# ucla-brain/image-preprocessing-pipeline

Hardware: AMD Instinct MI355X
Metric: RL-deconv Gvoxels/sec (higher is better)
Workload: dtype f32; 1 GPU; c3: 2048x2048x512 fp32 volume, 31x31x61 PSF, deconFFT semantics, lambda=0, reg_interval=0; engine=fft, parallelism=single

## Files before the change

image-preprocessing-pipeline_amd/csrc/fft_native_dev.h:

```cpp
#pragma once
#include <cmath>
#include <cstdlib>
#include <type_traits>
#include <vector>

#include "fft_native.h"

namespace mi {
namespace {

#ifndef MI_FFT_UNROLL
#define MI_FFT_UNROLL 4
#endif
#ifndef MI_YCUT
#define MI_YCUT 1
#endif
constexpr int kYCut = MI_YCUT;

__host__ __device__ constexpr int swz_g(int t) { return ((t & 1) ? 15 : 0) ^ ((t & 2) ? 13 : 0) ^ ((t & 4) ? 25 : 0) ^ ((t & 8) ? 16 : 0); }
__host__ __device__ constexpr int swz_c(int i) { return i ^ swz_g((i >> 4) & 15); }
__host__ __device__ constexpr unsigned long long swz_table_hi() {
    unsigned long long v = 0;
    for (int t = 0; t < 8; ++t) v |= (unsigned long long)swz_g(2 * t) << (5 * t);
    return v;
}
__device__ __forceinline__ int phys(int i) {
    constexpr unsigned long long T = swz_table_hi();
    const int hi = (int)((T >> (5 * ((i >> 5) & 7))) & 31ull);
    return i ^ hi ^ (__builtin_amdgcn_sbfe(i, 4, 1) & 15);
}
constexpr int kRowsRot = 256;
__device__ __forceinline__ int rmask(int row, int hp) {
    if (hp & kRowsRot) return (row >> 1) & ((hp & (kRowsRot - 1)) - 1);
    const int rp = (row >> 1) & (hp - 1);
    const int s = hp == 8 ? 1 : hp == 4 ? 2 : hp == 2 ? 3 : 0;
    return (rp << s) ^ ((rp & 1) << 4);
}

__device__ __forceinline__ int launder(int x) {
    asm volatile("" : "+v"(x));
    return x;
}
__device__ __forceinline__ void lds_barrier() {
    __builtin_amdgcn_fence(__ATOMIC_RELEASE, "workgroup", "local");
    __builtin_amdgcn_s_barrier();
    __builtin_amdgcn_fence(__ATOMIC_ACQUIRE, "workgroup", "local");
}
__device__ __forceinline__ void wave_lds_fence() {
    __builtin_amdgcn_fence(__ATOMIC_RELEASE, "wavefront", "local");
    __builtin_amdgcn_fence(__ATOMIC_ACQUIRE, "wavefront", "local");
}

__device__ __forceinline__ void stage_sync(bool priv) {
    if (priv) wave_lds_fence();
    else lds_barrier();
}

__device__ __forceinline__ float rcp_eps(float c) { return __builtin_amdgcn_rcpf(fmaxf(c, kEpsSingle)); }

typedef float v2f __attribute__((ext_vector_type(2)));
__device__ __forceinline__ v2f V2(float2 a) { return v2f{a.x, a.y}; }
__device__ __forceinline__ float2 F2(v2f a) { return make_float2(a.x, a.y); }
__device__ __forceinline__ float2 cmul(float2 a, float2 b) {
    const v2f A = V2(a), B = V2(b);
    const v2f axx = __builtin_shufflevector(A, A, 0, 0), ayy = __builtin_shufflevector(A, A, 1, 1);
    const v2f bs = {-B.y, B.x};
    return F2(__builtin_elementwise_fma(ayy, bs, axx * B));
}
__device__ __forceinline__ float2 cmulc(float2 a, float2 b) {
    const v2f A = V2(a), B = V2(b);
    const v2f axx = __builtin_shufflevector(A, A, 0, 0), ayy = __builtin_shufflevector(A, A, 1, 1);
    const v2f bc = {B.x, -B.y}, bsw = {B.y, B.x};
    return F2(__builtin_elementwise_fma(ayy, bsw, axx * bc));
}
__device__ __forceinline__ float2 cadd(float2 a, float2 b) { return F2(V2(a) + V2(b)); }
__device__ __forceinline__ float2 csub(float2 a, float2 b) { return F2(V2(a) - V2(b)); }
__device__ __forceinline__ float2 cconj(float2 a) { return make_float2(a.x, -a.y); }
__device__ __forceinline__ unsigned brev_n(unsigned v, int bits) { return bits == 0 ? 0u : (__brev(v) >> (32 - bits)); }

__device__ __forceinline__ int pos2freq(int p, int l2, int r3) {
    const int k1 = p >> l2, pp = p & ((1 << l2) - 1);
    return k1 + r3 * (int)brev_n((unsigned)pp, l2);
}
__device__ __forceinline__ int freq2pos(int k, int l2, int r3) {
    const int k2 = k / r3, k1 = k - k2 * r3;
    return (k1 << l2) + (int)brev_n((unsigned)k2, l2);
// ... 280 lines not shown
            dft3<INVERSE>(v[0], v[1], v[2]);
        } else if constexpr (R3 == 5) {
            dft5<INVERSE>(v);
        } else {
            if constexpr (!INVERSE) {
#pragma unroll
                for (int r = 0; r < 3; ++r) dft3<false>(v[r], v[r + 3], v[r + 6]);
                const float c9[3] = {1.0f, 0.76604444311897801f, 0.17364817766693033f};
                const float s9[3] = {0.0f, 0.64278760968653933f, 0.98480775301220802f};
                const float c94 = -0.93969262078590843f, s94 = 0.34202014332566871f;
                v[4] = cmul(v[4], make_float2(c9[1], -s9[1]));
                v[7] = cmul(v[7], make_float2(c9[2], -s9[2]));
                v[5] = cmul(v[5], make_float2(c9[2], -s9[2]));
                v[8] = cmul(v[8], make_float2(c94, -s94));
#pragma unroll
                for (int k1 = 0; k1 < 3; ++k1) dft3<false>(v[3 * k1], v[3 * k1 + 1], v[3 * k1 + 2]);
                float2 t[9];
#pragma unroll
                for (int k1 = 0; k1 < 3; ++k1)
#pragma unroll
                    for (int k2 = 0; k2 < 3; ++k2) t[k1 + 3 * k2] = v[3 * k1 + k2];
#pragma unroll
                for (int q = 0; q < 9; ++q) v[q] = t[q];
            } else {
                float2 t[9];
#pragma unroll
                for (int k1 = 0; k1 < 3; ++k1)
#pragma unroll
                    for (int k2 = 0; k2 < 3; ++k2) t[3 * k1 + k2] = v[k1 + 3 * k2];
#pragma unroll
                for (int q = 0; q < 9; ++q) v[q] = t[q];
#pragma unroll
                for (int k1 = 0; k1 < 3; ++k1) dft3<true>(v[3 * k1], v[3 * k1 + 1], v[3 * k1 + 2]);
                const float c9[3] = {1.0f, 0.76604444311897801f, 0.17364817766693033f};
                const float s9[3] = {0.0f, 0.64278760968653933f, 0.98480775301220802f};
                const float c94 = -0.93969262078590843f, s94 = 0.34202014332566871f;
                v[4] = cmul(v[4], make_float2(c9[1], s9[1]));
                v[7] = cmul(v[7], make_float2(c9[2], s9[2]));
                v[5] = cmul(v[5], make_float2(c9[2], s9[2]));
                v[8] = cmul(v[8], make_float2(c94, s94));
#pragma unroll
                for (int r = 0; r < 3; ++r) dft3<true>(v[r], v[r + 3], v[r + 6]);
            }
        }
        if (!INVERSE) {
#pragma unroll
            for (int q = 1; q < R3; ++q) v[q] = cmul(v[q], wq[q]);
        }
#pragma unroll
        for (int q = 0; q < R3; ++q) row[s0 ^ swz_c(q * msub)] = v[q];
    }
}

__device__ __forceinline__ int cell(int row, int pitch, int hp, int e) { return row * pitch + (phys(e) ^ rmask(row, hp)); }

template <class K, class... Args>
int launch_lds(K kernel, unsigned grid, int threads, size_t lds, hipStream_t s, const char* name, Args... args) {
    if (lds > 64 * 1024)
        MI_HIP(hipFuncSetAttribute(reinterpret_cast<const void*>(kernel), hipFuncAttributeMaxDynamicSharedMemorySize, (int)lds));
    hipLaunchKernelGGL(kernel, dim3(grid), dim3(threads), lds, s, args...);
    return launch_check(name);
}

template <int V>
using Int = std::integral_constant<int, V>;
#define MI_CASE_CALL(LG, R) case LG * 16 + R: return f(Int<LG>{}, Int<R>{});
template <class F>
int x_case(const NativeDims& d, F&& f) {
    switch (d.lhx2 * 16 + d.r3x) { MI_AXIS_CASES(MI_CASE_CALL) default: return fail(MI_ERR_UNSUPPORTED, "native FFT: x length %d", 2 * d.hx); }
}
template <class F>
int y_case(const NativeDims& d, F&& f) {
    switch (d.ly2 * 16 + d.r3) { MI_Y_CASES(MI_CASE_CALL) default: return fail(MI_ERR_UNSUPPORTED, "native FFT: y length %d", d.ny); }
}
#undef MI_CASE_CALL
#define MI_CASE_CALL(LG, R) case LG * 16 + R: if constexpr (axis_takes(2, LG, R)) return f(Int<LG>{}, Int<R>{}); else break;
template <class F>
int z_case(const NativeDims& d, F&& f) {
    switch (d.lz2 * 16 + d.r3z) { MI_AXIS_CASES(MI_CASE_CALL) default: break; }
    return fail(MI_ERR_UNSUPPORTED, "native FFT: z length %d", d.nz);
}
#undef MI_CASE_CALL

}
}
```

image-preprocessing-pipeline_amd/csrc/fft_native_yz.hip:

```cpp
#include "fft_native_dev.h"

namespace mi {
namespace {

template <int LY2, int R3, bool INVERSE>
__global__ __launch_bounds__(kThreadsY, 4) void k_y_pass(const float2* __restrict__ src, float2* __restrict__ dst, NativeDims d,
                                                      const float2* __restrict__ tw) {
    extern __shared__ __attribute__((aligned(16))) float2 tile[];
    constexpr int M = R3 << LY2, NW = kThreadsY / 64;
    constexpr int pitch = row_pitch(M), quads = M / 2;
    constexpr int TCC = y_tile_cols(M);
    const int TC = d.tc, Hx = d.hx, L = d.nz;
    const size_t c0 = (size_t)blockIdx.x * TC + (INVERSE ? (size_t)0 : (size_t)d.yz0 * Hx);
    if (!INVERSE) {
        if ((int)(c0 / Hx) >= d.z_in_hi) return;
    } else if (L % TC == 0) {
        const int z_first = (int)(c0 % L);
        if (z_first >= d.z_out_hi || z_first + TC <= d.z_out_lo) return;
    }
    const size_t src_pitch = INVERSE ? (size_t)M : (size_t)d.xrow, dst_pitch = INVERSE ? (size_t)d.xrow : (size_t)M;
    const float4* base = reinterpret_cast<const float4*>(src + c0 * src_pitch);
    const bool priv = (TC % NW) == 0;
    using TW = TwLds<LY2, R3, kYCut>;
    float2* twl = tile + TC * pitch;
// ... 34 lines not shown
        radix3_stage<R3, false, kThreadsY>(tile, TC, pitch, 1, priv, 1 << LY2, twl + TW::r3);
        stage_sync(priv);
    }
    lds_fft<LY2, INVERSE, kThreadsY, R3, 0, LY2, kYCut>(tile, TC * R3, pitch, 1, priv, twl);
    if constexpr (INVERSE && R3 > 1) {
        radix3_stage<R3, true, kThreadsY>(tile, TC, pitch, 1, priv, 1 << LY2, twl + TW::r3);
        stage_sync(priv);
    }
    if (fast) {
        const int s_lane = phys(2 * (int)threadIdx.x);
#pragma unroll
        for (int k = 0; k < NIT; ++k) {
            const int c = (k * kThreadsY) / quads, qk = (k * kThreadsY) % quads;
            const int s0 = c * pitch + (s_lane ^ swz_c(2 * qk));
            const float2 a = tile[s0], b = tile[s0 ^ 1];
            float4* dcol = reinterpret_cast<float4*>(dst + dest_col(c0 + c) * dst_pitch);
            if (!INVERSE || 2 * (qk + (int)threadIdx.x) < d.y_out_hi) dcol[qk + threadIdx.x] = make_float4(a.x, a.y, b.x, b.y);
        }
    } else {
#pragma unroll MI_FFT_UNROLL
        for (int i = first; i < n_items; i += step) {
            const int cl = i / quads, q = i - cl * quads;
            const int c = priv ? cl * NW + wave : cl;
            const int s0 = c * pitch + phys(2 * q);
            const float2 a = tile[s0], b = tile[s0 ^ 1];
            if (!INVERSE || 2 * q < d.y_out_hi) reinterpret_cast<float4*>(dst + dest_col(c0 + c) * dst_pitch)[q] = make_float4(a.x, a.y, b.x, b.y);
        }
    }
}

template <int LY2, int R3, bool INVERSE>
__global__ __launch_bounds__(kThreadsY, 4) void k_y_pair(const float2* __restrict__ src, float2* __restrict__ dst, NativeDims d,
                                                      const float2* __restrict__ tw) {
    extern __shared__ __attribute__((aligned(16))) float2 tile[];
    constexpr int M = R3 << LY2, NW = kThreadsY / 64;
    constexpr int pitch = row_pitch(M), quads = M / 2;
    const int TC = d.tc, Hx = d.hx, L = d.nz;
    const int zper = TC / 2, zblocks = L / zper, nxk = d.xkn;
    const int xkl = INVERSE ? blockIdx.x / zblocks : blockIdx.x % nxk;
    const int xk = d.xk0 + xkl;
    const int z0 = (INVERSE ? blockIdx.x - xkl * zblocks : blockIdx.x / nxk) * zper + (INVERSE ? 0 : d.yz0);
    if (!INVERSE) {
        if (z0 >= d.z_in_hi) return;
    } else if (z0 >= d.z_out_hi || z0 + zper <= d.z_out_lo) {
        return;
    }
    const int pxA = x_freq2pos(xk, d), pxB = x_freq2pos(xk == 0 ? 0 : Hx - xk, d);
    const bool self = pxA == pxB;
    auto x_item = [&](int i, int& c, int& q, size_t& g) {
        c = i / quads;
        q = i - c * quads;
        g = (((size_t)(z0 + (c >> 1)) * Hx + ((c & 1) ? pxB : pxA)) * d.xrow) / 2 + q;
    };
    auto z_item = [&](int i, int& c, int& s0, size_t& g) {
        const int zi = i / M, f = i - zi * M;
        const int py = ((f >> 3) << 3) + 2 * (f & 3), side = (f >> 2) & 1;
        c = 2 * zi + side;
        s0 = c * pitch + phys(!INVERSE && side ? mirror_pos(py, M, LY2, R3) : py);
        g = ((size_t)xk * L + z0 + zi) * (size_t)(M + d.zpad) + f;
    };
    auto x_slots = [&](int c, int q, int& s_lo, int& s_hi) {
        if (INVERSE && (c & 1)) {
            s_lo = c * pitch + phys(q == 0 ? 0 : M - 2 * q);
            s_hi = c * pitch + phys(M - 2 * q - 1);
        } else {
            s_lo = c * pitch + phys(2 * q);
            s_hi = s_lo ^ 1;
        }
    };
    const bool priv = (TC % NW) == 0;
    using TW = TwLds<LY2, R3, kYCut>;
    float2* twl = tile + TC * pitch;
    TW::template fill<kThreadsY>(twl, tw);
    const int n_items = TC * quads;
    constexpr int TCC = y_tile_cols(M);
    constexpr bool FAST_OK = R3 == 1 && quads % kThreadsY == 0;
    constexpr int NIT = FAST_OK ? TCC * quads / kThreadsY : 1;
    const bool fast = FAST_OK && TC == TCC;
    constexpr int WHI = FAST_OK ? LY2 - 9 : 0;
    static_assert(kThreadsY == 512, "the fast path of k_y_pair counts on 512 lanes");
    struct ZLane { int a, b0, b1, side; };
    auto z_lane = [&]() {
        const int tid = launder(threadIdx.x);
        const int py_l = ((tid >> 3) << 3) + 2 * (tid & 3), side = (tid >> 2) & 1;
        return ZLane{phys(py_l), phys(mirror_pos(py_l, M, LY2, R3)), phys(py_l ^ 511), side};
    };
    auto z_slot_fast = [&](const ZLane& zl, int k) {
        const int zi = (k * kThreadsY) / M, f0 = (k * kThreadsY) % M;
        const int flo = (int)brev_n((unsigned)f0, LY2);
        const int mhi = flo ? (int)brev_n((unsigned)((1 << WHI) - flo), LY2) : 0;
        const int sa = zl.a ^ swz_c(f0), sb = flo ? (zl.b1 ^ swz_c(mhi)) : zl.b0;
        return (2 * zi) * pitch + (zl.side ? pitch + sb : sa);
    };
    if (fast) {
        if (INVERSE) {
            const ZLane zl = z_lane();
            const float4* rowp = reinterpret_cast<const float4*>(src) + ((size_t)xk * L + z0) * (size_t)(M + d.zpad) + threadIdx.x;
#pragma unroll
            for (int k = 0; k < NIT; ++k) {
                const float4 v = rowp[(size_t)((k * kThreadsY) / M) * (M + d.zpad) + (k * kThreadsY) % M];
                const int s0 = z_slot_fast(zl, k);
                tile[s0] = make_float2(v.x, v.y);
                tile[s0 ^ 1] = make_float2(v.z, v.w);
            }
        } else {
            const int s_lane = phys(2 * (int)threadIdx.x);
#pragma unroll
            for (int k = 0; k < NIT; ++k) {
                const int c = (k * kThreadsY) / quads, qk = (k * kThreadsY) % quads;
                const size_t col = (((size_t)(z0 + (c >> 1)) * Hx + ((c & 1) ? pxB : pxA)) * d.xrow) / 2;
                const float4 v = reinterpret_cast<const float4*>(src)[col + qk + threadIdx.x];
                const int s0 = c * pitch + (s_lane ^ swz_c(2 * qk));
                tile[s0] = make_float2(v.x, v.y);
                tile[s0 ^ 1] = make_float2(v.z, v.w);
            }
        }
    } else {
#pragma unroll MI_FFT_UNROLL
    for (int i = threadIdx.x; i < n_items; i += kThreadsY) {
        int c, s0, s1;
        size_t g;
        if (INVERSE) {
            z_item(i, c, s0, g);
            s1 = s0 ^ 1;
        } else {
            int q;
            x_item(i, c, q, g);
            x_slots(c, q, s0, s1);
        }
        const float4 v = reinterpret_cast<const float4*>(src)[g];
        tile[s0] = make_float2(v.x, v.y);
        tile[s1] = make_float2(v.z, v.w);
    }
    }
    lds_barrier();
    if constexpr (!INVERSE && R3 > 1) {
        radix3_stage<R3, false, kThreadsY>(tile, TC, pitch, 1, priv, 1 << LY2, twl + TW::r3);
        stage_sync(priv);
    }
    lds_fft<LY2, INVERSE, kThreadsY, R3, 0, LY2, kYCut>(tile, TC * R3, pitch, 1, priv, twl);
    if constexpr (INVERSE && R3 > 1) {
        radix3_stage<R3, true, kThreadsY>(tile, TC, pitch, 1, priv, 1 << LY2, twl + TW::r3);
        stage_sync(priv);
    }
    if (priv) lds_barrier();
    if (fast) {
        if (INVERSE) {
            const int s_lane = phys(2 * (int)threadIdx.x);
#pragma unroll
            for (int k = 0; k < NIT; ++k) {
                const int c = (k * kThreadsY) / quads, qk = (k * kThreadsY) % quads;
                const int z = z0 + (c >> 1);
                if ((self && (c & 1)) || 2 * (qk + (int)threadIdx.x) >= d.y_out_hi || z < d.z_out_lo || z >= d.z_out_hi) continue;
                const size_t col = (((size_t)z * Hx + ((c & 1) ? pxB : pxA)) * d.xrow) / 2;
                const int s0 = c * pitch + (s_lane ^ swz_c(2 * qk));
                const float2 a = tile[s0], b = tile[s0 ^ 1];
                reinterpret_cast<float4*>(dst)[col + qk + threadIdx.x] = make_float4(a.x, a.y, b.x, b.y);
            }
        } else {
            const ZLane zl = z_lane();
            float4* rowp = reinterpret_cast<float4*>(dst) + ((size_t)xk * L + z0) * (size_t)(M + d.zpad) + threadIdx.x;
#pragma unroll
            for (int k = 0; k < NIT; ++k) {
                const int s0 = z_slot_fast(zl, k);
                const float2 a = tile[s0], b = tile[s0 ^ 1];
                rowp[(size_t)((k * kThreadsY) / M) * (M + d.zpad) + (k * kThreadsY) % M] = make_float4(a.x, a.y, b.x, b.y);
            }
        }
        return;
    }
#pragma unroll MI_FFT_UNROLL
    for (int i = threadIdx.x; i < n_items; i += kThreadsY) {
        int c, s0, s1;
        size_t g;
        if (INVERSE) {
            int q;
            x_item(i, c, q, g);
            const int z = z0 + (c >> 1);
            if ((self && (c & 1)) || 2 * q >= d.y_out_hi || z < d.z_out_lo || z >= d.z_out_hi) continue;
            x_slots(c, q, s0, s1);
        } else {
            z_item(i, c, s0, g);
            s1 = s0 ^ 1;
        }
        const float2 a = tile[s0], b = tile[s1];
        reinterpret_cast<float4*>(dst)[g] = make_float4(a.x, a.y, b.x, b.y);
    }
}

int y_launch(const NativeFft& f, hipStream_t s, bool inverse, YRoute route, unsigned ycols, const NativeDims& d, const float2* src, float2* dst) {
    const size_t yl = lds_bytes(d.tc, d.ny);
    return y_case(d, [&](auto lg, auto r) {
        constexpr int LG = lg(), R = r();
        if (route == YRoute::pair)
            return inverse ? launch_lds(k_y_pair<LG, R, true>, ycols, kThreadsY, yl, s, "k_y_pair<inv>", src, dst, d, f.tw_y)
                           : launch_lds(k_y_pair<LG, R, false>, ycols, kThreadsY, yl, s, "k_y_pair<fwd>", src, dst, d, f.tw_y);
        return inverse ? launch_lds(k_y_pass<LG, R, true>, ycols, kThreadsY, yl, s, "k_y_pass<inv>", src, dst, d, f.tw_y)
                       : launch_lds(k_y_pass<LG, R, false>, ycols, kThreadsY, yl, s, "k_y_pass<fwd>", src, dst, d, f.tw_y);
    });
}


template <int LZ2, int R3, bool BUILD>
__global__ __launch_bounds__(kThreadsXZ, kWavesXZ) void k_z_conv(const float2* __restrict__ S, float2* __restrict__ T, const float4* __restrict__ G,
                                                      NativeDims d, const float2* __restrict__ tw, int conj_otf, float4* __restrict__ Gout,
                                                      float scale) {
    extern __shared__ __attribute__((aligned(16))) float2 tile[];
    constexpr int L = R3 << LZ2, NW = kThreadsXZ / 64;
    const int Hx = d.hx, M = d.ny, TL = d.tl, hp = TL / 2, pitch = row_pitch(L);
    const int ytiles = M / TL;
    const int plane = blockIdx.x / ytiles;
    const int py0 = (blockIdx.x % ytiles) * TL;
    const int xk = plane;
    const int px = x_freq2pos(xk, d);
    const int pxB = x_freq2pos(xk == 0 ? 0 : Hx - xk, d);
    const int pyB_any = y_mirror_pos(py0, d);
    const int pyB0 = pyB_any & ~(TL - 1);
    const bool self_plane = (px == pxB);
    const float4* sA = reinterpret_cast<const float4*>(S + (size_t)px * L * M + py0);
    const float4* sB = reinterpret_cast<const float4*>(S + (size_t)pxB * L * M + pyB0);
    const int rowq = M / 2;
#pragma unroll MI_FFT_UNROLL
    for (int i = threadIdx.x; i < hp * L; i += kThreadsXZ) {
        const int z = i / hp, jp = i - z * hp;
        float4 a = make_float4(0.0f, 0.0f, 0.0f, 0.0f), b = a;
        if (z < d.z_in_hi) { a = sA[(size_t)z * rowq + jp]; b = sB[(size_t)z * rowq + jp]; }
        const int cA = cell(2 * jp, pitch, hp, z), cB = cA + TL * pitch;
        tile[cA] = make_float2(a.x, a.y);
        tile[cA + pitch] = make_float2(a.z, a.w);
        tile[cB] = make_float2(b.x, b.y);
        tile[cB + pitch] = make_float2(b.z, b.w);
    }
    const float4* Gp = G + ((size_t)plane * M + py0) * L;
    using TW = TwLds<LZ2, R3>;
    float2* twl = tile + 2 * TL * pitch;
    TW::template fill<kThreadsXZ>(twl, tw);
    lds_barrier();
    const bool priv = ((2 * TL) % NW) == 0;
    if (!(d.dbg & 1)) {
// ... 246 lines not shown
                if constexpr (REALG) {
                    float2 P = cmul(ph_xz, ph_yk[k]);
                    if (conj_otf) P.y = -P.y;
                    const float2 XaP = cmul(Xa, P), XbP = cmul(Xb, P);
                    Ya = make_float2(XaP.x * gr[k].x, XaP.y * gr[k].x);
                    Yb = make_float2(XbP.x * gr[k].y, XbP.y * gr[k].y);
                } else {
                    float2 Ga = make_float2(gv[k].x, gv[k].y), Gb = make_float2(gv[k].z, gv[k].w);
                    if (conj_otf) { Ga.y = -Ga.y; Gb.y = -Gb.y; }
                    Ya = cmul(Xa, Ga);
                    Yb = cmul(Xb, Gb);
                }
                const float2 E2 = make_float2(0.5f * (Ya.x + Yb.x), 0.5f * (Ya.y + Yb.y));
                const float2 dY = csub(Ya, Yb);
                const float2 O2 = cmulc(make_float2(0.5f * dY.x, 0.5f * dY.y), wx);
                tile[cA] = make_float2(E2.x - O2.y, E2.y + O2.x);
                tile[cB] = make_float2(E2.x + O2.y, O2.x - E2.y);
            }
        }
        const int tn = t + gridDim.x;
        if (R3 != 9 && tn < ntiles) load_S(tn);
        if (WP) wave_lds_fence();
        else lds_barrier();
        lds_fft<LZ2, true, kThreadsXZ, R3>(tile, 2 * TL * R3, pitch, hp, PRIV, twl);
        if constexpr (R3 > 1) {
            radix3_stage<R3, true, kThreadsXZ>(tile, 2 * TL, pitch, hp, PRIV, 1 << LZ2, twl + TW::r3);
            stage_sync(PRIV);
        }
        if (R3 == 9 && tn < ntiles) load_S(tn);
        if (PRIV) lds_barrier();
        const bool self_plane = (w.px == w.pxB);
        const FView fv = f_view();
        float4* dA = reinterpret_cast<float4*>(T + (size_t)w.px * L * M + w.py0) + fv.off;
        float4* dB = reinterpret_cast<float4*>(T + (size_t)w.pxB * L * M + w.pyB0) + fv.off;
#pragma unroll
        for (int k = 0; k < NPA; ++k) {
            const int zk = fv.z0 + k * P;
            if ((NA % kThreadsXZ == 0 || (int)threadIdx.x + k * kThreadsXZ < NA) && zk >= d.z_out_lo && zk < d.z_out_hi) {
                const int cA = fv.row + (fv.slot ^ swz_c(k * P));
                int cB0 = cA + TL * pitch, cB1 = cB0 + pitch;
                if constexpr (WP) b_cells(ptab, fv.jp, fv.pz ^ swz_c(k * P), cB0, cB1);
                const float2 a0 = tile[cA], a1 = tile[cA + pitch];
                dA[(size_t)(k * P) * rowq] = make_float4(a0.x, a0.y, a1.x, a1.y);
                if (!self_plane) {
                    const float2 b0 = tile[cB0], b1 = tile[cB1];
                    dB[(size_t)(k * P) * rowq] = make_float4(b0.x, b0.y, b1.x, b1.y);
                }
            }
        }
        lds_barrier();
    }
}

template <int LZ2, int R3, bool REALG, int NT, int TL, bool PHL = true, bool TOPON = true>
__global__ __launch_bounds__(NT, (NT == 512 && (R3 << LZ2) > 576) ? 2 : kWavesXZ) void k_z_pair_pipe(const float2* __restrict__ S, float2* __restrict__ T, const float4* __restrict__ G,
                                                              NativeDims d, const float2* __restrict__ tw, int conj_otf, int ntiles, RealOtf ro,
                                                              int* __restrict__ tile_ctr) {
    extern __shared__ __attribute__((aligned(16))) float2 tile[];
    __shared__ int s_next_tile;
    constexpr int L = R3 << LZ2, NW = NT / 64, hp = TL, pitch = row_pitch(L);
    constexpr bool WP = TL == NW;
    static_assert((WP || (NW == 2 * TL && L % 128 == 0)) && L % 64 == 0 && (TL * L) % NT == 0, "one or two waves per line pair");
    constexpr int NPA = TL * L / NT;
    constexpr int P = NT / TL;
    constexpr int NPG = TL * L / NT;
    constexpr int TOPS = seg_below(LZ2, LZ2), TOPR = LZ2 - TOPS;
    constexpr bool TOPREG = TOPON && R3 == 1 && (1 << TOPS) == P && (1 << TOPR) == NPA;
    const int Hx = d.hx, M = d.ny, ytiles = M / TL;
    const size_t ZR = (size_t)(M + d.zpad);
    struct FView { int row, slot, z0; size_t off; };
    auto f_view = [&]() {
        const int tid = launder(threadIdx.x);
        const int z0 = tid / TL, jq = tid - z0 * TL;
        return FView{(2 * jq) * pitch, phys(z0) ^ rmask(2 * jq, hp), z0, (size_t)z0 * ZR + jq};
    };
    float4 pre[NPA];
    auto load_S = [&](int t) {
        const int pl = t / ytiles, ty = t - pl * ytiles, plane = d.xk0 + pl;
        const FView fv = f_view();
        const float4* sp = reinterpret_cast<const float4*>(S) + (size_t)plane * L * ZR + (size_t)ty * TL + fv.off;
#pragma unroll
        for (int k = 0; k < NPA; ++k) pre[k] = (fv.z0 + k * P < d.z_in_hi) ? sp[(size_t)(k * P) * ZR] : make_float4(0.0f, 0.0f, 0.0f, 0.0f);
    };
    using TW = TwLds<LZ2, R3>;
    float2* twl = tile + 2 * TL * pitch;
    TW::template fill<NT>(twl, tw);
    float2* phl = twl + TW::total;
    if constexpr (REALG && PHL) {
        for (int p = threadIdx.x; p < L; p += NT) phl[p] = ro.ph_z[pos2freq(p, LZ2, R3)];
    }
    const bool dyn = tile_ctr != nullptr;
    int t = blockIdx.x, tn = t + (int)gridDim.x;
    if (dyn) {
        if (threadIdx.x == 0) s_next_tile = atomicAdd(tile_ctr, 2);
        lds_barrier();
        t = __builtin_amdgcn_readfirstlane(s_next_tile);
        tn = t + 1;
    }
    if (t < ntiles) load_S(t);
    lds_barrier();
    for (; t < ntiles;) {
        int fetched = 0;
        if (dyn && threadIdx.x == 0) fetched = atomicAdd(tile_ctr, 1);
        const int pl_ = t / ytiles, py0 = (t - pl_ * ytiles) * TL, plane = d.xk0 + pl_;
        {
            const FView fv = f_view();
            if constexpr (TOPREG) {
                float2 v[NPA], u[NPA];
#pragma unroll
                for (int k = 0; k < NPA; ++k) { v[k] = make_float2(pre[k].x, pre[k].y); u[k] = make_float2(pre[k].z, pre[k].w); }
                butterflies<TOPR, TOPS, false>(v, twl + tw_off(LZ2, TOPS), fv.z0);
                butterflies<TOPR, TOPS, false>(u, twl + tw_off(LZ2, TOPS), fv.z0);
#pragma unroll
                for (int k = 0; k < NPA; ++k) {
                    const int c = fv.row + (fv.slot ^ swz_c(k * P));
                    tile[c] = v[k];
                    tile[c + pitch] = u[k];
                }
            } else {
#pragma unroll
            for (int k = 0; k < NPA; ++k) {
                const int c = fv.row + (fv.slot ^ swz_c(k * P));
                tile[c] = make_float2(pre[k].x, pre[k].y);
                tile[c + pitch] = make_float2(pre[k].z, pre[k].w);
            }
            }
        }
        const size_t g0 = ((size_t)plane * M + py0) * L;
        float4 gv[REALG ? 1 : NPG];
        float2 gr[REALG ? NPG : 1];
        float2 ph_xy = make_float2(1.0f, 0.0f);
        auto load_G = [&]() {
            const int tid = launder(threadIdx.x);
            const int wv = __builtin_amdgcn_readfirstlane(tid >> 6);
            const int line = WP ? wv : wv % TL, p0 = WP ? 0 : (wv / TL) * (L / 2);
            if constexpr (REALG) {
                ph_xy = cmul(ro.ph_x[plane], ro.ph_y[y_pos2freq(py0 + line, d)]);
            }
            const size_t gl = g0 + (size_t)line * L + p0 + (tid & 63);
#pragma unroll
            for (int k = 0; k < NPG; ++k) {
                if constexpr (REALG) gr[k] = ro.g[gl + 64 * k];
                else gv[k] = G[gl + 64 * k];
            }
        };
        constexpr bool LATE_G = !REALG && R3 == 1 && !TOPREG && LZ2 - seg_below(LZ2, LZ2) == 4;
        if (R3 != 9 && !LATE_G) load_G();
        lds_barrier();
        if constexpr (R3 > 1) {
            radix3_stage<R3, false, NT>(tile, 2 * TL, pitch, hp, true, 1 << LZ2, twl + TW::r3);
            wave_lds_fence();
        }
        if (R3 == 9) load_G();
        if constexpr (LATE_G) {
            lds_fft<LZ2, false, NT, R3, 0, 4>(tile, 2 * TL * R3, pitch, hp, true, twl);
            load_G();
            lds_fft<LZ2, false, NT, R3, 4, LZ2>(tile, 2 * TL * R3, pitch, hp, true, twl);
        } else {
            lds_fft<LZ2, false, NT, R3, TOPREG ? TOPR : 0>(tile, 2 * TL * R3, pitch, hp, true, twl);
        }
        if constexpr (!WP) lds_barrier();
        float sw, cw;
        sincospif(-2.0f * (float)plane / (float)(2 * Hx), &sw, &cw);
        const float2 wx = make_float2(cw, sw);
        {
            const int tid = launder(threadIdx.x);
            const int wv = __builtin_amdgcn_readfirstlane(tid >> 6);
            const int lane = tid & 63;
            const int line = WP ? wv : wv % TL, p0 = WP ? 0 : (wv / TL) * (L / 2);
            const int pA = phys(lane) ^ rmask(line, hp), pB1 = phys(lane ^ 63) ^ rmask(TL + line, hp);
            const int pB0 = phys(mirror_pos(lane, L, LZ2, R3)) ^ rmask(TL + line, hp);
#pragma unroll
            for (int k = 0; k < NPG; ++k) {
                const int hb = 64 * k + p0;
                const int cA = line * pitch + (pA ^ swz_c(hb));
                int cB;
                if constexpr (R3 == 1) {
                    const int flo = (int)brev_n((unsigned)hb, LZ2);
                    const int mhi = flo ? (int)brev_n((unsigned)((1 << (LZ2 - 6)) - flo), LZ2) : 0;
                    cB = (TL + line) * pitch + (flo ? (pB1 ^ swz_c(mhi)) : pB0);
                } else {
                    cB = (TL + line) * pitch + (phys(mirror_pos(lane + hb, L, LZ2, R3)) ^ rmask(TL + line, hp));
                }
                const float2 a = tile[cA];
                const float2 bc = cconj(tile[cB]);
                const float2 E = make_float2(0.5f * (a.x + bc.x), 0.5f * (a.y + bc.y));
                const float2 dlt = csub(a, bc);
                const float2 O = make_float2(0.5f * dlt.y, -0.5f * dlt.x);
                const float2 wO = cmul(wx, O);
                const float2 Xa = cadd(E, wO), Xb = csub(E, wO);
                float2 Ya, Yb;
                if constexpr (REALG) {
                    float2 Pq = cmul(ph_xy, PHL ? phl[lane + hb] : ro.ph_z[pos2freq(lane + hb, LZ2, R3)]);
                    if (conj_otf) Pq.y = -Pq.y;
                    const float2 XaP = cmul(Xa, Pq), XbP = cmul(Xb, Pq);
                    Ya = make_float2(XaP.x * gr[k].x, XaP.y * gr[k].x);
                    Yb = make_float2(XbP.x * gr[k].y, XbP.y * gr[k].y);
                } else {
                    float2 Ga = make_float2(gv[k].x, gv[k].y), Gb = make_float2(gv[k].z, gv[k].w);
                    if (conj_otf) { Ga.y = -Ga.y; Gb.y = -Gb.y; }
                    Ya = cmul(Xa, Ga);
                    Yb = cmul(Xb, Gb);
                }
                const float2 E2 = make_float2(0.5f * (Ya.x + Yb.x), 0.5f * (Ya.y + Yb.y));
                const float2 dY = csub(Ya, Yb);
                const float2 O2 = cmulc(make_float2(0.5f * dY.x, 0.5f * dY.y), wx);
                tile[cA] = make_float2(E2.x - O2.y, E2.y + O2.x);
                tile[cB] = make_float2(E2.x + O2.y, O2.x - E2.y);
            }
        }
        if (R3 != 9 && tn < ntiles) load_S(tn);
        if constexpr (WP) wave_lds_fence();
        else lds_barrier();
        lds_fft<LZ2, true, NT, R3, 0, TOPREG ? TOPS : LZ2>(tile, 2 * TL * R3, pitch, hp, true, twl);
        if constexpr (R3 > 1) {
            radix3_stage<R3, true, NT>(tile, 2 * TL, pitch, hp, true, 1 << LZ2, twl + TW::r3);
            wave_lds_fence();
        }
        if (R3 == 9 && tn < ntiles) load_S(tn);
        lds_barrier();
        {
            const FView fv = f_view();
            float4* dp = reinterpret_cast<float4*>(T) + (size_t)plane * L * ZR + (size_t)(py0 / TL) * TL + fv.off;
#pragma unroll
            for (int k = 0; k < NPA; ++k) {
                const int zk = fv.z0 + k * P;
                if constexpr (!TOPREG) {
                if (zk >= d.z_out_lo && zk < d.z_out_hi) {
                    const int c = fv.row + (fv.slot ^ swz_c(k * P));
                    const float2 a0 = tile[c], a1 = tile[c + pitch];
                    dp[(size_t)(k * P) * ZR] = make_float4(a0.x, a0.y, a1.x, a1.y);
                }
                }
            }
            if constexpr (TOPREG) {
                float2 v[NPA], u[NPA];
#pragma unroll
                for (int k = 0; k < NPA; ++k) {
                    const int c = fv.row + (fv.slot ^ swz_c(k * P));
                    v[k] = tile[c];
                    u[k] = tile[c + pitch];
                }
                butterflies<TOPR, TOPS, true>(v, twl + tw_off(LZ2, TOPS), fv.z0);
                butterflies<TOPR, TOPS, true>(u, twl + tw_off(LZ2, TOPS), fv.z0);
#pragma unroll
                for (int k = 0; k < NPA; ++k) {
                    const int zk = fv.z0 + k * P;
                    if (zk >= d.z_out_lo && zk < d.z_out_hi) dp[(size_t)(k * P) * ZR] = make_float4(v[k].x, v[k].y, u[k].x, u[k].y);
                }
            }
        }
        if (dyn && threadIdx.x == 0) s_next_tile = fetched;
        lds_barrier();
        t = tn;
        tn = dyn ? __builtin_amdgcn_readfirstlane(s_next_tile) : tn + (int)gridDim.x;
    }
}

__global__ __launch_bounds__(256) void k_g_to_real(const float4* __restrict__ G, float2* __restrict__ Gr, NativeDims d, RealOtf ro,
                                                    size_t total, unsigned* __restrict__ stats) {
    const int M = d.ny, L = d.nz;
    float max_im = 0.0f, max_re = 0.0f;
    for (size_t i = blockIdx.x * (size_t)blockDim.x + threadIdx.x; i < total; i += (size_t)gridDim.x * blockDim.x) {
        const int pz = (int)(i % L);
        const size_t r = i / L;
        const int py = (int)(r % M), xk = (int)(r / M);
        const float2 P = cmul(cmul(ro.ph_x[xk], ro.ph_y[y_pos2freq(py, d)]), ro.ph_z[pos2freq(pz, d.lz2, d.r3z)]);
        const float4 g = G[i];
        const float2 a = cmulc(make_float2(g.x, g.y), P), b = cmulc(make_float2(g.z, g.w), P);
        Gr[i] = make_float2(a.x, b.x);
        max_im = fmaxf(max_im, fmaxf(fabsf(a.y), fabsf(b.y)));
        max_re = fmaxf(max_re, fmaxf(fabsf(a.x), fabsf(b.x)));
    }
    atomicMax(&stats[0], __float_as_uint(max_im));
    atomicMax(&stats[1], __float_as_uint(max_re));
}

RealOtf real_otf_args(const NativeFft& f, bool adj_slot) {
    RealOtf ro{};
    ro.g = adj_slot ? f.Gr_adj.as<float2>() : f.Gr.as<float2>();
    ro.ph_x = f.ph.as<float2>();
    ro.ph_y = ro.ph_x + (f.dims.hx / 2 + 1);
    ro.ph_z = ro.ph_y + f.dims.ny;
    return ro;
}

#define MI_ZQ_CALL(LG, R, NTH, PH) case LG * 16 + R: return f(Int<LG>{}, Int<R>{}, Int<NTH>{}, std::bool_constant<PH>{});
template <class F>
int z_pair_case(const NativeDims& d, F&& f) {
    switch (d.lz2 * 16 + d.r3z) { MI_ZQ_CASES(MI_ZQ_CALL) default: return fail(MI_ERR_UNSUPPORTED, "native FFT: paired z length %d", d.nz); }
}
#undef MI_ZQ_CALL

}
// ... 154 lines not shown
```

Baseline: 73.32 Gvoxel*iter/s.

## Move x-pair untangle into y pass and fuse radix-8 stage with OTF multiply

Moves the real-to-complex x-pair untangle/retangle step out of the z-pair pipeline and into the y pass's store and load paths. The z kernel's two packed columns then become independent rows (split layout with a new row mask), so the spectral multiply is a plain per-element product. For long z lines, it also fuses the last forward radix-8 stage, the OTF multiply and the first inverse radix-8 stage in registers, which saves LDS round trips. The cost is extra arithmetic in the y pass, a new LDS layout and a reordered phase table, all of which risk correctness and register pressure.

```diff
diff --git a/image-preprocessing-pipeline_amd/csrc/fft_native_dev.h b/image-preprocessing-pipeline_amd/csrc/fft_native_dev.h
--- a/image-preprocessing-pipeline_amd/csrc/fft_native_dev.h
+++ b/image-preprocessing-pipeline_amd/csrc/fft_native_dev.h
@@ -29,9 +29,10 @@
     const int hi = (int)((T >> (5 * ((i >> 5) & 7))) & 31ull);
     return i ^ hi ^ (__builtin_amdgcn_sbfe(i, 4, 1) & 15);
 }
-constexpr int kRowsRot = 256;
+constexpr int kRowsRot = 256, kRowsSplit = 512;
 __device__ __forceinline__ int rmask(int row, int hp) {
     if (hp & kRowsRot) return (row >> 1) & ((hp & (kRowsRot - 1)) - 1);
+    if (hp & kRowsSplit) return ((row & 7) << 1) ^ ((row & 1) << 4);
     const int rp = (row >> 1) & (hp - 1);
     const int s = hp == 8 ? 1 : hp == 4 ? 2 : hp == 2 ? 3 : 0;
     return (rp << s) ^ ((rp & 1) << 4);
@@ -418,6 +419,28 @@
     }
 }
 
+__device__ __forceinline__ float4 untangle_pair(float2 a, float2 b, float2 w) {
+    const v2f A = V2(a), Bc = {b.x, -b.y};
+    const v2f s = A + Bc, dlt = A - Bc;
+    const v2f O = {dlt.y, -dlt.x};
+    const v2f wO = __builtin_elementwise_fma(v2f{w.y, w.y}, dlt, v2f{w.x, w.x} * O);
+    const v2f Xa = s + wO, Xb = s - wO;
+    return make_float4(Xa.x, Xa.y, Xb.x, Xb.y);
+}
+__device__ __forceinline__ void retangle_pair(float4 y, float2 wq, float2& a, float2& b) {
+    const v2f Ya = {y.x, y.y}, Yb = {y.z, y.w};
+    const v2f s = Ya + Yb, dY = Ya - Yb;
+    const float2 O2 = cmul(F2(dY), wq);
+    a = F2(__builtin_elementwise_fma(s, v2f{0.25f, 0.25f}, v2f{-O2.y, O2.x}));
+    b = F2(__builtin_elementwise_fma(s, v2f{0.25f, -0.25f}, v2f{O2.y, O2.x}));
+}
+__device__ __forceinline__ float2 retangle_w(float2 w) { return make_float2(0.25f * w.x, -0.25f * w.y); }
+__device__ __forceinline__ float2 untangle_w(int xk, int hx) {
+    float sw, cw;
+    sincospif(-2.0f * (float)xk / (float)(2 * hx), &sw, &cw);
+    return make_float2(cw, sw);
+}
+
 __device__ __forceinline__ int cell(int row, int pitch, int hp, int e) { return row * pitch + (phys(e) ^ rmask(row, hp)); }
 
 template <class K, class... Args>
diff --git a/image-preprocessing-pipeline_amd/csrc/fft_native_yz.hip b/image-preprocessing-pipeline_amd/csrc/fft_native_yz.hip
--- a/image-preprocessing-pipeline_amd/csrc/fft_native_yz.hip
+++ b/image-preprocessing-pipeline_amd/csrc/fft_native_yz.hip
@@ -110,12 +110,11 @@
         q = i - c * quads;
         g = (((size_t)(z0 + (c >> 1)) * Hx + ((c & 1) ? pxB : pxA)) * d.xrow) / 2 + q;
     };
-    auto z_item = [&](int i, int& c, int& s0, size_t& g) {
-        const int zi = i / M, f = i - zi * M;
-        const int py = ((f >> 3) << 3) + 2 * (f & 3), side = (f >> 2) & 1;
-        c = 2 * zi + side;
-        s0 = c * pitch + phys(!INVERSE && side ? mirror_pos(py, M, LY2, R3) : py);
-        g = ((size_t)xk * L + z0 + zi) * (size_t)(M + d.zpad) + f;
+    auto z_item = [&](int i, int& sa, int& sb, size_t& g) {
+        const int zi = i / M, py = i - zi * M;
+        sa = (2 * zi) * pitch + phys(py);
+        sb = (2 * zi + 1) * pitch + phys(INVERSE ? py : mirror_pos(py, M, LY2, R3));
+        g = ((size_t)xk * L + z0 + zi) * (size_t)(M + d.zpad) + py;
     };
     auto x_slots = [&](int c, int q, int& s_lo, int& s_hi) {
         if (INVERSE && (c & 1)) {
@@ -137,29 +136,31 @@
     const bool fast = FAST_OK && TC == TCC;
     constexpr int WHI = FAST_OK ? LY2 - 9 : 0;
     static_assert(kThreadsY == 512, "the fast path of k_y_pair counts on 512 lanes");
-    struct ZLane { int a, b0, b1, side; };
+    struct ZLane { int a, b0, b1; };
     auto z_lane = [&]() {
         const int tid = launder(threadIdx.x);
-        const int py_l = ((tid >> 3) << 3) + 2 * (tid & 3), side = (tid >> 2) & 1;
-        return ZLane{phys(py_l), phys(mirror_pos(py_l, M, LY2, R3)), phys(py_l ^ 511), side};
-    };
-    auto z_slot_fast = [&](const ZLane& zl, int k) {
+        return ZLane{phys(tid), phys(mirror_pos(tid, M, LY2, R3)), phys(tid ^ 511)};
+    };
+    auto z_slots_fast = [&](const ZLane& zl, int k, int& sa, int& sb) {
         const int zi = (k * kThreadsY) / M, f0 = (k * kThreadsY) % M;
         const int flo = (int)brev_n((unsigned)f0, LY2);
         const int mhi = flo ? (int)brev_n((unsigned)((1 << WHI) - flo), LY2) : 0;
-        const int sa = zl.a ^ swz_c(f0), sb = flo ? (zl.b1 ^ swz_c(mhi)) : zl.b0;
-        return (2 * zi) * pitch + (zl.side ? pitch + sb : sa);
+        sa = (2 * zi) * pitch + (zl.a ^ swz_c(f0));
+        sb = (2 * zi + 1) * pitch + (flo ? (zl.b1 ^ swz_c(mhi)) : zl.b0);
     };
     if (fast) {
         if (INVERSE) {
+            const float4* rowp = reinterpret_cast<const float4*>(src) + ((size_t)xk * L + z0) * (size_t)(M + d.zpad) + threadIdx.x;
+            float4 v[NIT];
+#pragma unroll
+            for (int k = 0; k < NIT; ++k) v[k] = rowp[(size_t)((k * kThreadsY) / M) * (M + d.zpad) + (k * kThreadsY) % M];
             const ZLane zl = z_lane();
-            const float4* rowp = reinterpret_cast<const float4*>(src) + ((size_t)xk * L + z0) * (size_t)(M + d.zpad) + threadIdx.x;
+            const float2 wq = retangle_w(untangle_w(xk, Hx));
 #pragma unroll
             for (int k = 0; k < NIT; ++k) {
-                const float4 v = rowp[(size_t)((k * kThreadsY) / M) * (M + d.zpad) + (k * kThreadsY) % M];
-                const int s0 = z_slot_fast(zl, k);
-                tile[s0] = make_float2(v.x, v.y);
-                tile[s0 ^ 1] = make_float2(v.z, v.w);
+                int sa, sb;
+                z_slots_fast(zl, k, sa, sb);
+                retangle_pair(v[k], wq, tile[sa], tile[sb]);
             }
         } else {
             const int s_lane = phys(2 * (int)threadIdx.x);
@@ -174,21 +175,22 @@
             }
         }
     } else {
+    const float2 wx = INVERSE ? retangle_w(untangle_w(xk, Hx)) : make_float2(1.0f, 0.0f);
 #pragma unroll MI_FFT_UNROLL
     for (int i = threadIdx.x; i < n_items; i += kThreadsY) {
         int c, s0, s1;
         size_t g;
         if (INVERSE) {
-            z_item(i, c, s0, g);
-            s1 = s0 ^ 1;
+            z_item(i, s0, s1, g);
+            retangle_pair(reinterpret_cast<const float4*>(src)[g], wx, tile[s0], tile[s1]);
         } else {
             int q;
             x_item(i, c, q, g);
             x_slots(c, q, s0, s1);
-        }
-        const float4 v = reinterpret_cast<const float4*>(src)[g];
-        tile[s0] = make_float2(v.x, v.y);
-        tile[s1] = make_float2(v.z, v.w);
+            const float4 v = reinterpret_cast<const float4*>(src)[g];
+            tile[s0] = make_float2(v.x, v.y);
+            tile[s1] = make_float2(v.z, v.w);
+        }
     }
     }
     lds_barrier();
@@ -217,16 +219,18 @@
             }
         } else {
             const ZLane zl = z_lane();
+            const float2 wx = untangle_w(xk, Hx);
             float4* rowp = reinterpret_cast<float4*>(dst) + ((size_t)xk * L + z0) * (size_t)(M + d.zpad) + threadIdx.x;
 #pragma unroll
             for (int k = 0; k < NIT; ++k) {
-                const int s0 = z_slot_fast(zl, k);
-                const float2 a = tile[s0], b = tile[s0 ^ 1];
-                rowp[(size_t)((k * kThreadsY) / M) * (M + d.zpad) + (k * kThreadsY) % M] = make_float4(a.x, a.y, b.x, b.y);
+                int sa, sb;
+                z_slots_fast(zl, k, sa, sb);
+                rowp[(size_t)((k * kThreadsY) / M) * (M + d.zpad) + (k * kThreadsY) % M] = untangle_pair(tile[sa], tile[sb], wx);
             }
         }
         return;
     }
+    const float2 wx = INVERSE ? make_float2(1.0f, 0.0f) : untangle_w(xk, Hx);
 #pragma unroll MI_FFT_UNROLL
     for (int i = threadIdx.x; i < n_items; i += kThreadsY) {
         int c, s0, s1;
@@ -237,12 +241,12 @@
             const int z = z0 + (c >> 1);
             if ((self && (c & 1)) || 2 * q >= d.y_out_hi || z < d.z_out_lo || z >= d.z_out_hi) continue;
             x_slots(c, q, s0, s1);
+            const float2 a = tile[s0], b = tile[s1];
+            reinterpret_cast<float4*>(dst)[g] = make_float4(a.x, a.y, b.x, b.y);
         } else {
-            z_item(i, c, s0, g);
-            s1 = s0 ^ 1;
-        }
-        const float2 a = tile[s0], b = tile[s1];
-        reinterpret_cast<float4*>(dst)[g] = make_float4(a.x, a.y, b.x, b.y);
+            z_item(i, s0, s1, g);
+            reinterpret_cast<float4*>(dst)[g] = untangle_pair(tile[s0], tile[s1], wx);
+        }
     }
 }
 
@@ -595,27 +599,31 @@
     }
 }
 
-template <int LZ2, int R3, bool REALG, int NT, int TL, bool PHL = true, bool TOPON = true>
+template <int LZ2, int R3, bool REALG, int NT, int TL, bool PHL = true, bool TOPON = true, bool FUSEON = true>
 __global__ __launch_bounds__(NT, (NT == 512 && (R3 << LZ2) > 576) ? 2 : kWavesXZ) void k_z_pair_pipe(const float2* __restrict__ S, float2* __restrict__ T, const float4* __restrict__ G,
                                                               NativeDims d, const float2* __restrict__ tw, int conj_otf, int ntiles, RealOtf ro,
                                                               int* __restrict__ tile_ctr) {
     extern __shared__ __attribute__((aligned(16))) float2 tile[];
     __shared__ int s_next_tile;
-    constexpr int L = R3 << LZ2, NW = NT / 64, hp = TL, pitch = row_pitch(L);
-    constexpr bool WP = TL == NW;
-    static_assert((WP || (NW == 2 * TL && L % 128 == 0)) && L % 64 == 0 && (TL * L) % NT == 0, "one or two waves per line pair");
+    constexpr int L = R3 << LZ2, NW = NT / 64, hp = kRowsSplit | TL, pitch = row_pitch(L);
+    static_assert(TL == 8, "the row masks of the split float4 (rmask, kRowsSplit) are those of eight rows");
+    static_assert((2 * TL) % NW == 0 && L % 64 == 0 && (TL * L) % NT == 0, "whole rows per wave");
+    constexpr int NR = 2 * TL / NW, NI = L / 64;
+    constexpr bool WP = NR == 2;
+    static_assert(WP || NR == 1, "a wave owns a line pair or one line");
+    constexpr bool FUSE = FUSEON && R3 == 1 && WP && LZ2 >= 9;
+    static_assert(!FUSE || (PHL && seg_r(LZ2, 0) == 3), "the fused stage is the radix-8 bottom stage and keeps the LDS phase table");
     constexpr int NPA = TL * L / NT;
     constexpr int P = NT / TL;
-    constexpr int NPG = TL * L / NT;
     constexpr int TOPS = seg_below(LZ2, LZ2), TOPR = LZ2 - TOPS;
     constexpr bool TOPREG = TOPON && R3 == 1 && (1 << TOPS) == P && (1 << TOPR) == NPA;
-    const int Hx = d.hx, M = d.ny, ytiles = M / TL;
+    const int M = d.ny, ytiles = M / TL;
     const size_t ZR = (size_t)(M + d.zpad);
     struct FView { int row, slot, z0; size_t off; };
     auto f_view = [&]() {
         const int tid = launder(threadIdx.x);
         const int z0 = tid / TL, jq = tid - z0 * TL;
-        return FView{(2 * jq) * pitch, phys(z0) ^ rmask(2 * jq, hp), z0, (size_t)z0 * ZR + jq};
+        return FView{jq * pitch, phys(z0) ^ rmask(jq, hp), z0, (size_t)z0 * ZR + jq};
     };
     float4 pre[NPA];
     auto load_S = [&](int t) {
@@ -630,7 +638,7 @@
     TW::template fill<NT>(twl, tw);
     float2* phl = twl + TW::total;
     if constexpr (REALG && PHL) {
-        for (int p = threadIdx.x; p < L; p += NT) phl[p] = ro.ph_z[pos2freq(p, LZ2, R3)];
+        for (int p = threadIdx.x; p < L; p += NT) phl[FUSE ? (((p >> 9) * 8 + (p & 7)) * 64 + ((p >> 3) & 63)) : p] = ro.ph_z[pos2freq(p, LZ2, R3)];
     }
     const bool dyn = tile_ctr != nullptr;
     int t = blockIdx.x, tn = t + (int)gridDim.x;
@@ -658,33 +666,49 @@
                 for (int k = 0; k < NPA; ++k) {
                     const int c = fv.row + (fv.slot ^ swz_c(k * P));
                     tile[c] = v[k];
-                    tile[c + pitch] = u[k];
+                    tile[c + TL * pitch] = u[k];
                 }
             } else {
 #pragma unroll
             for (int k = 0; k < NPA; ++k) {
                 const int c = fv.row + (fv.slot ^ swz_c(k * P));
                 tile[c] = make_float2(pre[k].x, pre[k].y);
-                tile[c + pitch] = make_float2(pre[k].z, pre[k].w);
+                tile[c + TL * pitch] = make_float2(pre[k].z, pre[k].w);
             }
             }
         }
         const size_t g0 = ((size_t)plane * M + py0) * L;
-        float4 gv[REALG ? 1 : NPG];
-        float2 gr[REALG ? NPG : 1];
+        float4 g4[!REALG && WP ? NI : 1];
+        float2 g2[REALG == WP ? NI : 1];
+        float g1[REALG && !WP ? NI : 1];
         float2 ph_xy = make_float2(1.0f, 0.0f);
         auto load_G = [&]() {
             const int tid = launder(threadIdx.x);
             const int wv = __builtin_amdgcn_readfirstlane(tid >> 6);
-            const int line = WP ? wv : wv % TL, p0 = WP ? 0 : (wv / TL) * (L / 2);
-            if constexpr (REALG) {
-                ph_xy = cmul(ro.ph_x[plane], ro.ph_y[y_pos2freq(py0 + line, d)]);
-            }
-            const size_t gl = g0 + (size_t)line * L + p0 + (tid & 63);
-#pragma unroll
-            for (int k = 0; k < NPG; ++k) {
-                if constexpr (REALG) gr[k] = ro.g[gl + 64 * k];
-                else gv[k] = G[gl + 64 * k];
+            const int line = wv % TL, side = wv / TL;
+            if constexpr (REALG) ph_xy = cmul(ro.ph_x[plane], ro.ph_y[y_pos2freq(py0 + line, d)]);
+            if constexpr (FUSE) {
+                const size_t g8 = g0 + (size_t)line * L + 8 * (tid & 63);
+#pragma unroll
+                for (int q = 0; q < NI; q += 2) {
+                    if constexpr (REALG) {
+                        const float4 v = reinterpret_cast<const float4*>(ro.g + g8)[256 * (q >> 3) + (q & 7) / 2];
+                        g2[q] = make_float2(v.x, v.y);
+                        g2[q + 1] = make_float2(v.z, v.w);
+                    } else {
+                        g4[q] = G[g8 + 512 * (q >> 3) + (q & 7)];
+                        g4[q + 1] = G[g8 + 512 * (q >> 3) + (q & 7) + 1];
+                    }
+                }
+                return;
+            }
+            const size_t gl = g0 + (size_t)line * L + (tid & 63);
+#pragma unroll
+            for (int k = 0; k < NI; ++k) {
+                if constexpr (REALG && WP) g2[k] = ro.g[gl + 64 * k];
+                else if constexpr (REALG) g1[k] = reinterpret_cast<const float*>(ro.g)[2 * (gl + 64 * k) + side];
+                else if constexpr (WP) g4[k] = G[gl + 64 * k];
+                else g2[k] = reinterpret_cast<const float2*>(G)[2 * (gl + 64 * k) + side];
             }
         };
         constexpr bool LATE_G = !REALG && R3 == 1 && !TOPREG && LZ2 - seg_below(LZ2, LZ2) == 4;
@@ -698,64 +722,85 @@
         if constexpr (LATE_G) {
             lds_fft<LZ2, false, NT, R3, 0, 4>(tile, 2 * TL * R3, pitch, hp, true, twl);
             load_G();
-            lds_fft<LZ2, false, NT, R3, 4, LZ2>(tile, 2 * TL * R3, pitch, hp, true, twl);
+            lds_fft<LZ2, false, NT, R3, 4, FUSE ? LZ2 - 3 : LZ2>(tile, 2 * TL * R3, pitch, hp, true, twl);
         } else {
-            lds_fft<LZ2, false, NT, R3, TOPREG ? TOPR : 0>(tile, 2 * TL * R3, pitch, hp, true, twl);
-        }
-        if constexpr (!WP) lds_barrier();
-        float sw, cw;
-        sincospif(-2.0f * (float)plane / (float)(2 * Hx), &sw, &cw);
-        const float2 wx = make_float2(cw, sw);
-        {
+            lds_fft<LZ2, false, NT, R3, TOPREG ? TOPR : 0, FUSE ? LZ2 - 3 : LZ2>(tile, 2 * TL * R3, pitch, hp, true, twl);
+        }
+        if constexpr (FUSE) {
             const int tid = launder(threadIdx.x);
             const int wv = __builtin_amdgcn_readfirstlane(tid >> 6);
-            const int lane = tid & 63;
-            const int line = WP ? wv : wv % TL, p0 = WP ? 0 : (wv / TL) * (L / 2);
-            const int pA = phys(lane) ^ rmask(line, hp), pB1 = phys(lane ^ 63) ^ rmask(TL + line, hp);
-            const int pB0 = phys(mirror_pos(lane, L, LZ2, R3)) ^ rmask(TL + line, hp);
-#pragma unroll
-            for (int k = 0; k < NPG; ++k) {
-                const int hb = 64 * k + p0;
-                const int cA = line * pitch + (pA ^ swz_c(hb));
-                int cB;
-                if constexpr (R3 == 1) {
-                    const int flo = (int)brev_n((unsigned)hb, LZ2);
-                    const int mhi = flo ? (int)brev_n((unsigned)((1 << (LZ2 - 6)) - flo), LZ2) : 0;
-                    cB = (TL + line) * pitch + (flo ? (pB1 ^ swz_c(mhi)) : pB0);
+            const int lane = tid & 63, x0 = phys(lane << 3) ^ rmask(wv, hp);
+#pragma unroll
+            for (int it = 0; it < NI / 8; ++it) {
+                const int c0 = wv * pitch + (x0 ^ swz_c(512 * it));
+                float2 Pq[REALG ? 8 : 1];
+                if constexpr (REALG) {
+#pragma unroll
+                    for (int j = 0; j < 8; ++j) {
+                        Pq[j] = cmul(ph_xy, phl[(8 * it + j) * 64 + lane]);
+                        if (conj_otf) Pq[j].y = -Pq[j].y;
+                    }
+                }
+#pragma unroll
+                for (int side = 0; side < 2; ++side) {
+                    float2* row = tile + side * TL * pitch;
+                    float2 v[8];
+#pragma unroll
+                    for (int j = 0; j < 8; ++j) v[j] = row[c0 ^ j];
+                    butterflies<3, 0, false>(v, twl, 0);
+#pragma unroll
+                    for (int j = 0; j < 8; ++j) {
+                        if constexpr (REALG) {
+                            const float2 vp = cmul(v[j], Pq[j]);
+                            const float g = side ? g2[8 * it + j].y : g2[8 * it + j].x;
+                            v[j] = make_float2(vp.x * g, vp.y * g);
+                        } else {
+                            const float4 g = g4[8 * it + j];
+                            float2 Gq = side ? make_float2(g.z, g.w) : make_float2(g.x, g.y);
+                            if (conj_otf) Gq.y = -Gq.y;
+                            v[j] = cmul(v[j], Gq);
+                        }
+                    }
+                    butterflies<3, 0, true>(v, twl, 0);
+#pragma unroll
+                    for (int j = 0; j < 8; ++j) row[c0 ^ j] = v[j];
+                }
+            }
+        } else {
+            const int tid = launder(threadIdx.x);
+            const int wv = __builtin_amdgcn_readfirstlane(tid >> 6);
+            const int lane = tid & 63, x0 = phys(lane) ^ rmask(wv, hp);
+#pragma unroll
+            for (int k = 0; k < NI; ++k) {
+                const int cA = wv * pitch + (x0 ^ swz_c(64 * k)), cB = cA + TL * pitch;
+                float2 Pq = make_float2(1.0f, 0.0f);
+                if constexpr (REALG) {
+                    Pq = cmul(ph_xy, PHL ? phl[lane + 64 * k] : ro.ph_z[pos2freq(lane + 64 * k, LZ2, R3)]);
+                    if (conj_otf) Pq.y = -Pq.y;
+                }
+                if constexpr (REALG && WP) {
+                    const float2 aP = cmul(tile[cA], Pq), bP = cmul(tile[cB], Pq);
+                    tile[cA] = make_float2(aP.x * g2[k].x, aP.y * g2[k].x);
+                    tile[cB] = make_float2(bP.x * g2[k].y, bP.y * g2[k].y);
+                } else if constexpr (REALG) {
+                    const float2 aP = cmul(tile[cA], Pq);
+                    tile[cA] = make_float2(aP.x * g1[k], aP.y * g1[k]);
+                } else if constexpr (WP) {
+                    float2 Ga = make_float2(g4[k].x, g4[k].y), Gb = make_float2(g4[k].z, g4[k].w);
+                    if (conj_otf) { Ga.y = -Ga.y; Gb.y = -Gb.y; }
+                    const float2 ya = cmul(tile[cA], Ga), yb = cmul(tile[cB], Gb);
+                    tile[cA] = ya;
+                    tile[cB] = yb;
                 } else {
-                    cB = (TL + line) * pitch + (phys(mirror_pos(lane + hb, L, LZ2, R3)) ^ rmask(TL + line, hp));
-                }
-                const float2 a = tile[cA];
-                const float2 bc = cconj(tile[cB]);
-                const float2 E = make_float2(0.5f * (a.x + bc.x), 0.5f * (a.y + bc.y));
-                const float2 dlt = csub(a, bc);
-                const float2 O = make_float2(0.5f * dlt.y, -0.5f * dlt.x);
-                const float2 wO = cmul(wx, O);
-                const float2 Xa = cadd(E, wO), Xb = csub(E, wO);
-                float2 Ya, Yb;
-                if constexpr (REALG) {
-                    float2 Pq = cmul(ph_xy, PHL ? phl[lane + hb] : ro.ph_z[pos2freq(lane + hb, LZ2, R3)]);
-                    if (conj_otf) Pq.y = -Pq.y;
-                    const float2 XaP = cmul(Xa, Pq), XbP = cmul(Xb, Pq);
-                    Ya = make_float2(XaP.x * gr[k].x, XaP.y * gr[k].x);
-                    Yb = make_float2(XbP.x * gr[k].y, XbP.y * gr[k].y);
-                } else {
-                    float2 Ga = make_float2(gv[k].x, gv[k].y), Gb = make_float2(gv[k].z, gv[k].w);
-                    if (conj_otf) { Ga.y = -Ga.y; Gb.y = -Gb.y; }
-                    Ya = cmul(Xa, Ga);
-                    Yb = cmul(Xb, Gb);
-                }
-                const float2 E2 = make_float2(0.5f * (Ya.x + Yb.x), 0.5f * (Ya.y + Yb.y));
-                const float2 dY = csub(Ya, Yb);
-                const float2 O2 = cmulc(make_float2(0.5f * dY.x, 0.5f * dY.y), wx);
-                tile[cA] = make_float2(E2.x - O2.y, E2.y + O2.x);
-                tile[cB] = make_float2(E2.x + O2.y, O2.x - E2.y);
+                    float2 Gq = g2[k];
+                    if (conj_otf) Gq.y = -Gq.y;
+                    tile[cA] = cmul(tile[cA], Gq);
+                }
             }
         }
         if (R3 != 9 && tn < ntiles) load_S(tn);
-        if constexpr (WP) wave_lds_fence();
-        else lds_barrier();
-        lds_fft<LZ2, true, NT, R3, 0, TOPREG ? TOPS : LZ2>(tile, 2 * TL * R3, pitch, hp, true, twl);
+        wave_lds_fence();
+        lds_fft<LZ2, true, NT, R3, FUSE ? 3 : 0, TOPREG ? TOPS : LZ2>(tile, 2 * TL * R3, pitch, hp, true, twl);
         if constexpr (R3 > 1) {
             radix3_stage<R3, true, NT>(tile, 2 * TL, pitch, hp, true, 1 << LZ2, twl + TW::r3);
             wave_lds_fence();
@@ -771,7 +816,7 @@
                 if constexpr (!TOPREG) {
                 if (zk >= d.z_out_lo && zk < d.z_out_hi) {
                     const int c = fv.row + (fv.slot ^ swz_c(k * P));
-                    const float2 a0 = tile[c], a1 = tile[c + pitch];
+                    const float2 a0 = tile[c], a1 = tile[c + TL * pitch];
                     dp[(size_t)(k * P) * ZR] = make_float4(a0.x, a0.y, a1.x, a1.y);
                 }
                 }
@@ -782,7 +827,7 @@
                 for (int k = 0; k < NPA; ++k) {
                     const int c = fv.row + (fv.slot ^ swz_c(k * P));
                     v[k] = tile[c];
-                    u[k] = tile[c + pitch];
+                    u[k] = tile[c + TL * pitch];
                 }
                 butterflies<TOPR, TOPS, true>(v, twl + tw_off(LZ2, TOPS), fv.z0);
                 butterflies<TOPR, TOPS, true>(u, twl + tw_off(LZ2, TOPS), fv.z0);
```

Result: slower. 72.27 Gvoxel*iter/s (-1.4%).
